# zhen6618/EPRecon

Measured on AMD Instinct MI355X. Metric: fragments_per_sec, higher is better.
Workload: dtype f32

## Files before the change

### eprecon_amd/csrc/back_project.hip

```cpp
#include <stdlib.h>

#include "common.hpp"

namespace {
using namespace ep;


struct BpParams {
    const int32_t *coords;
    int n;
    const float *origin;
    int batch;
    float voxel_size;
    const float *feats_nhwc;
    const float *krcam;
    int V, C, H, W;
    int Cs;
    int min_view;
    float *out_feats;
    float *out_mean;
    int32_t *out_coords;
    float *count;
    float *out_grid;
    uint8_t *out_mask;
    int32_t *n_valid_dev;
    int32_t *block_offsets;
    int xcd_slabs;
};

struct Proj {
    float gx, gy, pz;
    bool vis;
};

__device__ __forceinline__ Proj project(const float *P, float X, float Y, float Z, float wm1,
                                        float hm1)
{
    const float px = __fmaf_rn(P[3], 1.0f, __fmaf_rn(P[2], Z, __fmaf_rn(P[1], Y, __fmul_rn(P[0], X))));
    const float py = __fmaf_rn(P[7], 1.0f, __fmaf_rn(P[6], Z, __fmaf_rn(P[5], Y, __fmul_rn(P[4], X))));
    const float pz = __fmaf_rn(P[11], 1.0f, __fmaf_rn(P[10], Z, __fmaf_rn(P[9], Y, __fmul_rn(P[8], X))));
    const float u = __fdiv_rn(px, pz);
    const float v = __fdiv_rn(py, pz);
    Proj r;
    r.gx = __fsub_rn(__fdiv_rn(__fmul_rn(2.0f, u), wm1), 1.0f);
    r.gy = __fsub_rn(__fdiv_rn(__fmul_rn(2.0f, v), hm1), 1.0f);
    r.pz = pz;
    r.vis = (fabsf(r.gx) <= 1.0f) && (fabsf(r.gy) <= 1.0f) && (pz > 0.0f);
    return r;
}

struct ProjFast {
    float u, v, pz;
    bool vis;
};

__device__ __forceinline__ ProjFast project_fast(const float *P, float X, float Y, float Z, float wm1, float hm1,
                                                 float kx, float ky)
{
    const float px = __fmaf_rn(P[3], 1.0f, __fmaf_rn(P[2], Z, __fmaf_rn(P[1], Y, __fmul_rn(P[0], X))));
    const float py = __fmaf_rn(P[7], 1.0f, __fmaf_rn(P[6], Z, __fmaf_rn(P[5], Y, __fmul_rn(P[4], X))));
    const float pz = __fmaf_rn(P[11], 1.0f, __fmaf_rn(P[10], Z, __fmaf_rn(P[9], Y, __fmul_rn(P[8], X))));
    float r = __builtin_amdgcn_rcpf(pz);
    r = r * fmaf(-pz, r, 2.0f);
    const float u = px * r, v = py * r;
    const float gx = fmaf(u, kx, -1.0f), gy = fmaf(v, ky, -1.0f);
    ProjFast o;
    o.pz = pz;
    const bool near_edge = fabsf(fabsf(gx) - 1.0f) < 1e-4f || fabsf(fabsf(gy) - 1.0f) < 1e-4f;
    if (near_edge) {
        const float ue = __fdiv_rn(px, pz), ve = __fdiv_rn(py, pz);
        const float gxe = __fsub_rn(__fdiv_rn(__fmul_rn(2.0f, ue), wm1), 1.0f);
        const float gye = __fsub_rn(__fdiv_rn(__fmul_rn(2.0f, ve), hm1), 1.0f);
        o.vis = (fabsf(gxe) <= 1.0f) && (fabsf(gye) <= 1.0f) && (pz > 0.0f);
    } else {
        o.vis = (fabsf(gx) <= 1.0f) && (fabsf(gy) <= 1.0f) && (pz > 0.0f);
    }
    o.u = fminf(fmaxf(u, 0.0f), wm1);
    o.v = fminf(fmaxf(v, 0.0f), hm1);
    return o;
}

__device__ __forceinline__ void voxel_centre(const int4 c, const float *origin, float vs, float &X,
                                             float &Y, float &Z)
{
    X = __fadd_rn(__fmul_rn((float)c.y, vs), origin[3 * c.x + 0]);
    Y = __fadd_rn(__fmul_rn((float)c.z, vs), origin[3 * c.x + 1]);
    Z = __fadd_rn(__fmul_rn((float)c.w, vs), origin[3 * c.x + 2]);
}

__device__ __forceinline__ void stage_matrices(float *sP, const float *krcam, int nmat, int tid,
                                               int nthreads)
{
    for (int i = tid; i < nmat * 12; i += nthreads) {
        const int m = i / 12, e = i - m * 12;
        sP[i] = krcam[m * 16 + e];
    }
}

template <int VOX>
__global__ __launch_bounds__(256) void bp_count_kernel(BpParams p, int32_t *tile_sums, int32_t *blk_batch)
{
    constexpr int BLOCK = 256;
    extern __shared__ __attribute__((aligned(16))) char smem[];
    float *sP = reinterpret_cast<float *>(smem);
    int *sBatch = reinterpret_cast<int *>(sP + p.V * p.batch * 12);
    int *sWave = sBatch + p.batch;
    const int tid = threadIdx.x;
    stage_matrices(sP, p.krcam, p.V * p.batch, tid, BLOCK);
    for (int b = tid; b < p.batch; b += BLOCK) sBatch[b] = 0;
    __syncthreads();

    const int i = blockIdx.x * BLOCK + tid;
    bool valid = false;
    int vbatch = 0;
    if (i < p.n) {
        const int4 c = reinterpret_cast<const int4 *>(p.coords)[i];
        int cnt = 0;
        const bool in_range = c.x >= 0 && c.x < p.batch;
        if (in_range) {
            float X, Y, Z;
            voxel_centre(c, p.origin, p.voxel_size, X, Y, Z);
            const float wm1 = (float)(p.W - 1), hm1 = (float)(p.H - 1);
            const float kx = 2.0f / wm1, ky = 2.0f / hm1;
            for (int v = 0; v < p.V; ++v)
                cnt += project_fast(sP + (v * p.batch + c.x) * 12, X, Y, Z, wm1, hm1, kx, ky).vis ? 1 : 0;
        }
        p.count[i] = (float)cnt;
        valid = in_range && cnt >= p.min_view;
        vbatch = c.x;
    }
    const unsigned long long m = __ballot(valid);
    const int lane = tid & (kWave - 1);
    {
        const int b0 = __shfl(vbatch, m ? (__ffsll((long long)m) - 1) : 0);
        const bool uniform = __ballot(valid && vbatch != b0) == 0ull;
        if (uniform) {
            if (m && lane == (__ffsll((long long)m) - 1)) atomicAdd(&sBatch[b0], __popcll(m));
        } else if (valid) {
            atomicAdd(&sBatch[vbatch], 1);
        }
    }
    if constexpr (VOX >= kWave) {
        if (lane == 0) sWave[tid / kWave] = __popcll(m);
        __syncthreads();
        constexpr int WPT = VOX / kWave;
        if (tid < BLOCK / VOX) {
            int t = 0;
            for (int w = 0; w < WPT; ++w) t += sWave[tid * WPT + w];
            const int tile = blockIdx.x * (BLOCK / VOX) + tid;
            if ((long long)tile * VOX < p.n) tile_sums[tile] = t;
        }
    } else {
        if ((lane % VOX) == 0 && i < p.n) tile_sums[i / VOX] = __popcll((m >> lane) & ((1ull << VOX) - 1ull));
        __syncthreads();
    }
    if (blk_batch) {
        __syncthreads();
        for (int b = tid; b < p.batch; b += BLOCK) blk_batch[(size_t)blockIdx.x * p.batch + b] = sBatch[b];
    }
}

__global__ __launch_bounds__(1024) void bp_scan_kernel(int32_t *block_sums, int nblk,
                                                       int32_t *n_valid_dev, const int32_t *blk_batch = nullptr,
                                                       int nblk_count = 0, int batch = 0)
{
    __shared__ int sWave[1024 / kWave];
    const int tid = threadIdx.x, lane = tid & (kWave - 1), wid = tid / kWave;
    int carry = 0;
    for (int base = 0; base < nblk; base += 1024) {
        const int i = base + tid;
        const int v = i < nblk ? block_sums[i] : 0;
        int x = v;
#pragma unroll
        for (int d = 1; d < kWave; d <<= 1) {
            const int y = __shfl_up(x, d);
            if (lane >= d) x += y;
        }
        if (lane == kWave - 1) sWave[wid] = x;
        __syncthreads();
        int woff = 0, tot = 0;
#pragma unroll
        for (int w = 0; w < 1024 / kWave; ++w) {
            const int c = sWave[w];
            woff += (w < wid) ? c : 0;
            tot += c;
        }
        if (i < nblk) block_sums[i] = carry + woff + x - v;
        carry += tot;
        __syncthreads();
    }
    if (tid == 0) n_valid_dev[0] = carry;
    if (batch == 1) {
        if (tid == 0) n_valid_dev[1] = carry;
    } else if (blk_batch) {
        for (int b = 0; b < batch; ++b) {
            int x = 0;
            for (int i = tid; i < nblk_count; i += 1024) x += blk_batch[(size_t)i * batch + b];
#pragma unroll
            for (int d = kWave / 2; d > 0; d >>= 1) x += __shfl_xor(x, d);
            __syncthreads();
            if (lane == 0) sWave[wid] = x;
            __syncthreads();
            if (tid == 0) {
                int t = 0;
                for (int w = 0; w < 1024 / kWave; ++w) t += sWave[w];
                n_valid_dev[1 + b] = t;
            }
        }
    }
}

struct Taps {
    int o00, o10, o01, o11;
    float w00, w10, w01, w11;
};

__device__ __forceinline__ Taps make_taps(float ix, float iy, int W, int H, int C)
{
    const float x0f = floorf(ix), y0f = floorf(iy);
    int x0 = (int)x0f, y0 = (int)y0f;
    float wx1 = ix - x0f, wx0 = (x0f + 1.0f) - ix;
    float wy1 = iy - y0f, wy0 = (y0f + 1.0f) - iy;
    int x1 = x0 + 1, y1 = y0 + 1;
    if (x1 >= W) { x1 = W - 1; wx1 = 0.0f; }
    if (y1 >= H) { y1 = H - 1; wy1 = 0.0f; }
    Taps t;
    t.o00 = (y0 * W + x0) * C;
    t.o10 = (y0 * W + x1) * C;
    t.o01 = (y1 * W + x0) * C;
    t.o11 = (y1 * W + x1) * C;
    t.w00 = wx0 * wy0;
    t.w10 = wx1 * wy0;
    t.w01 = wx0 * wy1;
    t.w11 = wx1 * wy1;
    return t;
}

template <int VEC>
struct Chan;
template <>
struct Chan<4> {
    float4 v;
    __device__ __forceinline__ static Chan zero() { return Chan{make_float4(0.f, 0.f, 0.f, 0.f)}; }
    __device__ __forceinline__ static Chan sample(const float *m, const Taps &t)
    {
        const float4 a = *reinterpret_cast<const float4 *>(m + t.o00);
        const float4 b = *reinterpret_cast<const float4 *>(m + t.o10);
        const float4 c = *reinterpret_cast<const float4 *>(m + t.o01);
        const float4 d = *reinterpret_cast<const float4 *>(m + t.o11);
        Chan r;
        r.v.x = fmaf(d.x, t.w11, fmaf(c.x, t.w01, fmaf(b.x, t.w10, a.x * t.w00)));
        r.v.y = fmaf(d.y, t.w11, fmaf(c.y, t.w01, fmaf(b.y, t.w10, a.y * t.w00)));
        r.v.z = fmaf(d.z, t.w11, fmaf(c.z, t.w01, fmaf(b.z, t.w10, a.z * t.w00)));
        r.v.w = fmaf(d.w, t.w11, fmaf(c.w, t.w01, fmaf(b.w, t.w10, a.w * t.w00)));
        return r;
    }
    __device__ __forceinline__ void add(const Chan &o) { v.x += o.v.x; v.y += o.v.y; v.z += o.v.z; v.w += o.v.w; }
    __device__ __forceinline__ void add_sqdiff(const Chan &f, const Chan &mean)
    {
        const float dx = f.v.x - mean.v.x, dy = f.v.y - mean.v.y, dz = f.v.z - mean.v.z, dw = f.v.w - mean.v.w;
        v.x = fmaf(dx, dx, v.x); v.y = fmaf(dy, dy, v.y); v.z = fmaf(dz, dz, v.z); v.w = fmaf(dw, dw, v.w);
    }
    __device__ __forceinline__ Chan div(float d) const
    {
        return Chan{make_float4(__fdiv_rn(v.x, d), __fdiv_rn(v.y, d), __fdiv_rn(v.z, d), __fdiv_rn(v.w, d))};
    }
    __device__ __forceinline__ void store(float *dst, bool aligned16) const
    {
        if (aligned16) {
            *reinterpret_cast<float4 *>(dst) = v;
        } else {
            dst[0] = v.x; dst[1] = v.y; dst[2] = v.z; dst[3] = v.w;
        }
    }
};
template <>
struct Chan<1> {
    float v;
    __device__ __forceinline__ static Chan zero() { return Chan{0.f}; }
    __device__ __forceinline__ static Chan sample(const float *m, const Taps &t)
    {
        return Chan{fmaf(m[t.o11], t.w11, fmaf(m[t.o01], t.w01, fmaf(m[t.o10], t.w10, m[t.o00] * t.w00)))};
    }
    __device__ __forceinline__ void add(const Chan &o) { v += o.v; }
    __device__ __forceinline__ void add_sqdiff(const Chan &f, const Chan &mean)
    {
        const float d = f.v - mean.v;
        v = fmaf(d, d, v);
    }
    __device__ __forceinline__ Chan div(float d) const { return Chan{__fdiv_rn(v, d)}; }
    __device__ __forceinline__ void store(float *dst, bool) const { dst[0] = v; }
};

template <int VOX, int MODE, int VEC, int QT>
__global__ __launch_bounds__(256) void bp_gather_kernel(BpParams p)
{
    extern __shared__ __attribute__((aligned(16))) char smem[];
    constexpr int BLOCK = 256;
    float2 *sPix = reinterpret_cast<float2 *>(smem);
    float *sP = reinterpret_cast<float *>(sPix + VOX * p.V);
    const int nP = (p.V * p.batch * 12 + 3) & ~3;
    uint32_t *sVis = reinterpret_cast<uint32_t *>(sP + nP);
    float *sDen = reinterpret_cast<float *>(sVis + VOX);
    int *sBatch = reinterpret_cast<int *>(sDen + VOX);
    int *sSlot = sBatch + VOX;
    int *sOut = sSlot + VOX;
    int *sWave = sOut + VOX;

    const int tid = threadIdx.x;
    const int lb = p.xcd_slabs ? xcd_remap(blockIdx.x, gridDim.x) : (int)blockIdx.x;
    stage_matrices(sP, p.krcam, p.V * p.batch, tid, BLOCK);
    __syncthreads();

    const int e = lb * VOX + tid;
    const int i = e;
    const float wm1 = (float)(p.W - 1), hm1 = (float)(p.H - 1);
    bool valid = false;
    int4 c = make_int4(0, 0, 0, 0);
    float X = 0.f, Y = 0.f, Z = 0.f, zsum = 0.f;
    int cnt = 0;
    uint32_t vis = 0;
    if (tid < VOX && e < p.n) {
        c = reinterpret_cast<const int4 *>(p.coords)[i];
        if (c.x >= 0 && c.x < p.batch) {
            voxel_centre(c, p.origin, p.voxel_size, X, Y, Z);
            for (int v = 0; v < p.V; ++v) {
                const Proj pr = project(sP + (v * p.batch + c.x) * 12, X, Y, Z, wm1, hm1);
                const float ix = __fmul_rn(__fdiv_rn(__fadd_rn(pr.gx, 1.0f), 2.0f), wm1);
                const float iy = __fmul_rn(__fdiv_rn(__fadd_rn(pr.gy, 1.0f), 2.0f), hm1);
                sPix[tid * p.V + v] = make_float2(ix, iy);
                if (pr.vis) {
                    vis |= 1u << v;
                    cnt += 1;
                    zsum += pr.pz;
                }
            }
            valid = cnt >= p.min_view;
        }
    }
    int nloc;
    const int rank = block_exclusive_rank<BLOCK>(valid, sWave, nloc);
    if (nloc == 0) return;
    const int base = p.block_offsets[lb];
    const int n_valid = p.n_valid_dev[0];
    const int cout = (MODE == EPRECON_BP_MEAN_DEPTH) ? p.C + 1 : p.C;
    if (valid) {
        const int o = base + rank;
        sSlot[rank] = tid;
        sOut[tid] = o;
        sVis[tid] = vis;
        const float den = (float)(cnt > 0 ? cnt : 1);
        sDen[tid] = den;
        sBatch[tid] = c.x;
        reinterpret_cast<int4 *>(p.out_coords)[o] = c;
        if (MODE == EPRECON_BP_MEAN_DEPTH) p.out_feats[(size_t)o * cout + p.C] = __fdiv_rn(zsum, den);
        if (p.out_grid || p.out_mask) {
            for (int v = 0; v < p.V; ++v) {
                const Proj pr = project(sP + (v * p.batch + c.x) * 12, X, Y, Z, wm1, hm1);
                if (p.out_grid)
                    reinterpret_cast<float2 *>(p.out_grid)[(size_t)v * n_valid + o] = make_float2(pr.gx, pr.gy);
                if (p.out_mask) p.out_mask[(size_t)v * n_valid + o] = pr.vis ? 1 : 0;
            }
        }
    }
    __syncthreads();

    const int Q = QT > 0 ? QT : p.C / VEC;
    const size_t map_elems = (size_t)p.H * p.W * p.Cs;
    const bool aligned16 = (MODE != EPRECON_BP_MEAN_DEPTH);
    for (int w = tid; w < nloc * Q; w += BLOCK) {
        const int r = w / Q;
        const int q = w - r * Q;
        const int t = sSlot[r];
        const uint32_t vm = sVis[t];
        const float den = sDen[t];
        const int b = sBatch[t];
        const float *fb = p.feats_nhwc + (size_t)b * map_elems + q * VEC;
        const size_t vstride = (size_t)p.batch * map_elems;
        Chan<VEC> acc = Chan<VEC>::zero();
        for (int v = 0; v < p.V; ++v) {
            if (vm & (1u << v)) {
                const float2 px = sPix[t * p.V + v];
                const Taps tp = make_taps(px.x, px.y, p.W, p.H, p.Cs);
                acc.add(Chan<VEC>::sample(fb + (size_t)v * vstride, tp));
            }
        }
        const int orow = sOut[t];
        float *dst = p.out_feats + (size_t)orow * cout + q * VEC;
        if (MODE == EPRECON_BP_VARIANCE) {
            const Chan<VEC> mean = acc.div(den);
            Chan<VEC> sq = Chan<VEC>::zero();
            for (int v = 0; v < p.V; ++v) {
                if (vm & (1u << v)) {
                    const float2 px = sPix[t * p.V + v];
                    const Taps tp = make_taps(px.x, px.y, p.W, p.H, p.Cs);
                    sq.add_sqdiff(Chan<VEC>::sample(fb + (size_t)v * vstride, tp), mean);
                }
            }
            sq.div(den).store(dst, true);
            if (p.out_mean) mean.store(p.out_mean + (size_t)orow * p.C + q * VEC, true);
        } else {
            acc.div(den).store(dst, aligned16);
        }
    }
}


typedef unsigned int u32x4 __attribute__((ext_vector_type(4)));

constexpr int kOobOffset = (int)0x80000000u;

template <int U, class F>
__device__ __forceinline__ void visit_visible_samples(__amdgpu_buffer_rsrc_t rsrc, const int *sOffRow,
                                                      const float2 *sWxyRow, uint32_t vm, int qbyte, int s10,
                                                      int s01, int s11, F &&f)
{
    uint32_t m = vm;
    while (m) {
        int off[U];
        float2 wxy[U];
        bool on[U];
#pragma unroll
        for (int u = 0; u < U; ++u) {
            on[u] = m != 0;
            const int v = on[u] ? __builtin_ctz(m) : 0;
            m &= m - 1;
            wxy[u] = sWxyRow[v];
            off[u] = on[u] ? sOffRow[v] + qbyte : kOobOffset;
        }
        u32x4 a[U], b[U], c[U], d[U];
#pragma unroll
        for (int u = 0; u < U; ++u) {
            a[u] = __builtin_amdgcn_raw_buffer_load_b128(rsrc, off[u], 0, 0);
            b[u] = __builtin_amdgcn_raw_buffer_load_b128(rsrc, off[u], s10, 0);
            c[u] = __builtin_amdgcn_raw_buffer_load_b128(rsrc, off[u], s01, 0);
            d[u] = __builtin_amdgcn_raw_buffer_load_b128(rsrc, off[u], s11, 0);
        }
#pragma unroll
        for (int u = 0; u < U; ++u) {
            const float wx1 = wxy[u].x, wy1 = wxy[u].y;
            const float wx0 = 1.0f - wx1, wy0 = 1.0f - wy1;
            const float w00 = wx0 * wy0, w10 = wx1 * wy0, w01 = wx0 * wy1, w11 = wx1 * wy1;
            float4 r;
#define EP_TAP(k) fmaf(__uint_as_float(d[u].k), w11, fmaf(__uint_as_float(c[u].k), w01, fmaf(__uint_as_float(b[u].k), w10, __uint_as_float(a[u].k) * w00)))
            r.x = EP_TAP(x); r.y = EP_TAP(y); r.z = EP_TAP(z); r.w = EP_TAP(w);
#undef EP_TAP
            if (on[u]) f(r);
        }
    }
}

template <int VOX, int MODE, int QT, int U>
__global__ __launch_bounds__(256) void bp_gather_mlp_kernel(BpParams p)
{
    extern __shared__ __attribute__((aligned(16))) char smem[];
    constexpr int BLOCK = 256;
    constexpr int VPT = BLOCK / VOX;
    float2 *sWxy = reinterpret_cast<float2 *>(smem);
    int *sOff = reinterpret_cast<int *>(sWxy + VOX * p.V);
    float *sP = reinterpret_cast<float *>(sOff + VOX * p.V);
    const int nP = (p.V * p.batch * 12 + 3) & ~3;
    uint32_t *sVis = reinterpret_cast<uint32_t *>(sP + nP);
    int *sSlot = reinterpret_cast<int *>(sVis + VOX);
    int *sOut = sSlot + VOX;
    int *sWave = sOut + VOX;

    const int tid = threadIdx.x;
    const int lb = p.xcd_slabs ? xcd_remap(blockIdx.x, gridDim.x) : (int)blockIdx.x;
    stage_matrices(sP, p.krcam, p.V * p.batch, tid, BLOCK);
    if (VPT > 1 && tid < VOX) sVis[tid] = 0;
    __syncthreads();

    const float wm1 = (float)(p.W - 1), hm1 = (float)(p.H - 1);
    const float kx = 2.0f / wm1, ky = 2.0f / hm1;
    const int map_elems = p.H * p.W * p.Cs;
    const int vx = tid % VOX;
    const int e = lb * VOX + vx;
    int4 c = make_int4(-1, 0, 0, 0);
    if (e < p.n) c = reinterpret_cast<const int4 *>(p.coords)[e];
    const bool in_batch = c.x >= 0 && c.x < p.batch;
    uint32_t vis = 0;
    if (in_batch) {
        float X, Y, Z;
        voxel_centre(c, p.origin, p.voxel_size, X, Y, Z);
        for (int v = tid / VOX; v < p.V; v += VPT) {
            const ProjFast q = project_fast(sP + (v * p.batch + c.x) * 12, X, Y, Z, wm1, hm1, kx, ky);
            if (!q.vis) continue;
            const float x0f = fminf(floorf(q.u), wm1 - 1.0f), y0f = fminf(floorf(q.v), hm1 - 1.0f);
            sWxy[vx * p.V + v] = make_float2(q.u - x0f, q.v - y0f);
            sOff[vx * p.V + v] = ((v * p.batch + c.x) * map_elems + ((int)y0f * p.W + (int)x0f) * p.Cs) * 4;
            vis |= 1u << v;
        }
        if (VPT > 1 && vis) atomicOr(&sVis[vx], vis);
    }
    if (VPT > 1) {
        __syncthreads();
        vis = sVis[vx];
    }
    const int cnt = __popc(vis);
    const bool valid = tid < VOX && in_batch && cnt >= p.min_view;
    int nloc;
    const int rank = block_exclusive_rank<BLOCK>(valid, sWave, nloc);
    if (nloc == 0) return;
    const int n_valid = p.n_valid_dev[0];
    const int cout = (MODE == EPRECON_BP_MEAN_DEPTH) ? p.C + 1 : p.C;
    if (valid) {
        const int o = p.block_offsets[lb] + rank;
        sSlot[rank] = tid;
        sOut[tid] = o;
        if (VPT == 1) sVis[tid] = vis;
        reinterpret_cast<int4 *>(p.out_coords)[o] = c;
        if (MODE == EPRECON_BP_MEAN_DEPTH || p.out_grid || p.out_mask) {
            float X, Y, Z, zsum = 0.0f;
            voxel_centre(c, p.origin, p.voxel_size, X, Y, Z);
            for (int v = 0; v < p.V; ++v) {
                const Proj pr = project(sP + (v * p.batch + c.x) * 12, X, Y, Z, wm1, hm1);
                if (pr.vis) zsum += pr.pz;
                if (p.out_grid)
                    reinterpret_cast<float2 *>(p.out_grid)[(size_t)v * n_valid + o] = make_float2(pr.gx, pr.gy);
                if (p.out_mask) p.out_mask[(size_t)v * n_valid + o] = pr.vis ? 1 : 0;
            }
            if (MODE == EPRECON_BP_MEAN_DEPTH)
                p.out_feats[(size_t)o * cout + p.C] = __fdiv_rn(zsum, (float)(cnt > 0 ? cnt : 1));
        }
    }
    __syncthreads();
    const __amdgpu_buffer_rsrc_t rsrc = __builtin_amdgcn_make_buffer_rsrc(
        const_cast<float *>(p.feats_nhwc), 0, p.V * p.batch * map_elems * 4, 0x00020000);
    const int Q = QT > 0 ? QT : p.C / 4;
    const int s10 = p.Cs * 4, s01 = p.W * p.Cs * 4, s11 = s01 + s10;
    for (int w = tid; w < nloc * Q; w += BLOCK) {
        const int r = w / Q, q = w - r * Q;
        const int t = sSlot[r];
        const uint32_t vm = sVis[t];
        const float den = (float)max(__popc(vm), 1);
        const int *offRow = sOff + t * p.V;
        const float2 *wxyRow = sWxy + t * p.V;
        float4 acc = make_float4(0.f, 0.f, 0.f, 0.f);
        visit_visible_samples<U>(rsrc, offRow, wxyRow, vm, q * 16, s10, s01, s11, [&](const float4 &f) {
            acc.x += f.x; acc.y += f.y; acc.z += f.z; acc.w += f.w;
        });
        const int orow = sOut[t];
        float *dst = p.out_feats + (size_t)orow * cout + q * 4;
        const float4 mean = make_float4(__fdiv_rn(acc.x, den), __fdiv_rn(acc.y, den), __fdiv_rn(acc.z, den),
                                        __fdiv_rn(acc.w, den));
        if (MODE == EPRECON_BP_VARIANCE) {
            float4 sq = make_float4(0.f, 0.f, 0.f, 0.f);
            visit_visible_samples<U>(rsrc, offRow, wxyRow, vm, q * 16, s10, s01, s11, [&](const float4 &f) {
                const float dx = f.x - mean.x, dy = f.y - mean.y, dz = f.z - mean.z, dw = f.w - mean.w;
                sq.x = fmaf(dx, dx, sq.x); sq.y = fmaf(dy, dy, sq.y); sq.z = fmaf(dz, dz, sq.z); sq.w = fmaf(dw, dw, sq.w);
            });
            *reinterpret_cast<float4 *>(dst) = make_float4(__fdiv_rn(sq.x, den), __fdiv_rn(sq.y, den),
                                                           __fdiv_rn(sq.z, den), __fdiv_rn(sq.w, den));
            if (p.out_mean) *reinterpret_cast<float4 *>(p.out_mean + (size_t)orow * p.C + q * 4) = mean;
        } else if (MODE == EPRECON_BP_MEAN_DEPTH) {
            dst[0] = mean.x; dst[1] = mean.y; dst[2] = mean.z; dst[3] = mean.w;
        } else {
            *reinterpret_cast<float4 *>(dst) = mean;
        }
    }
}


__global__ __launch_bounds__(1024) void bp_depth_norm_kernel(float *out_feats, int cout,
                                                             const int32_t *n_valid_dev)
{
    __shared__ float sRed[1024 / kWave];
    __shared__ float sBcast[2];
    const int b = blockIdx.x, tid = threadIdx.x, lane = tid & (kWave - 1), wid = tid / kWave;
    int start = 0;
    for (int k = 0; k < b; ++k) start += n_valid_dev[1 + k];
    const int len = n_valid_dev[1 + b];
    float *d = out_feats + (size_t)start * cout + (cout - 1);

    auto block_sum = [&](float x) -> float {
#pragma unroll
        for (int s = kWave / 2; s > 0; s >>= 1) x += __shfl_xor(x, s);
        __syncthreads();
        if (lane == 0) sRed[wid] = x;
        __syncthreads();
        float t = 0.f;
#pragma unroll
        for (int w = 0; w < 1024 / kWave; ++w) t += sRed[w];
        return t;
    };
    float s = 0.f, m = 0.f;
    for (int j = tid; j < len; j += 1024) {
        const float x = d[(size_t)j * cout];
        if (x > 0.f) { s += x; m += 1.f; }
    }
    const float tot = block_sum(s), cntp = block_sum(m);
    const float mu = tot / cntp;
    float ss = 0.f;
    for (int j = tid; j < len; j += 1024) {
        const float x = d[(size_t)j * cout];
        if (x > 0.f) ss = fmaf(x - mu, x - mu, ss);
    }
    const float sigma = sqrtf(block_sum(ss)) + 1e-5f;
    for (int j = tid; j < len; j += 1024) {
        const float x = d[(size_t)j * cout];
        d[(size_t)j * cout] = x > 0.f ? (x - mu) / sigma : 0.f;
    }
    (void)sBcast;
}

constexpr int kTrPix = 64;
__global__ __launch_bounds__(256) void nchw_to_nhwc_kernel(const float *__restrict__ in,
                                                           float *__restrict__ out, int C, int hw, int Cs,
                                                           int32_t *zero = nullptr, int zero_n = 0)
{
    extern __shared__ __attribute__((aligned(16))) char smem[];
    float *tile = reinterpret_cast<float *>(smem);
    if (blockIdx.x == 0 && blockIdx.y == 0 && (int)threadIdx.x < zero_n) zero[threadIdx.x] = 0;
    const int map = blockIdx.y;
    const int p0 = blockIdx.x * kTrPix;
    const int npix = min(kTrPix, hw - p0);
    const float *src = in + (size_t)map * C * hw;
    float *dst = out + (size_t)map * hw * Cs + (size_t)p0 * Cs;
    for (int e = threadIdx.x; e < C * kTrPix; e += 256) {
        const int c = e / kTrPix, px = e - c * kTrPix;
        if (px < npix) tile[c * (kTrPix + 1) + px] = src[(size_t)c * hw + p0 + px];
    }
    __syncthreads();
    for (int e = threadIdx.x; e < npix * Cs; e += 256) {
        const int px = e / Cs, c = e - px * Cs;
        dst[e] = c < C ? tile[c * (kTrPix + 1) + px] : 0.0f;
    }
}


struct ViewsParams {
    eprecon_views_desc d;
    int tile0[4];
    int tiles[3];
};
__global__ __launch_bounds__(256) void views_to_rows_kernel(ViewsParams p)
{
    extern __shared__ __attribute__((aligned(16))) char smem[];
    float *tile = reinterpret_cast<float *>(smem);
    const int b = blockIdx.x;
    const int l = b >= p.tile0[2] ? 2 : (b >= p.tile0[1] ? 1 : 0);
    const int r = b - p.tile0[l];
    const int v = r / p.tiles[l], t = r - v * p.tiles[l];
    const int C = p.d.channels[l], hw = p.d.hw[l];
    const int p0 = t * kTrPix;
    const int npix = min(kTrPix, hw - p0);
    const float *src = p.d.src[l][v];
    float *dst = p.d.dst[l] + ((size_t)v * hw + p0) * C;
    for (int e = threadIdx.x; e < C * kTrPix; e += 256) {
        const int c = e / kTrPix, px = e - c * kTrPix;
        if (px < npix) tile[c * (kTrPix + 1) + px] = src[(size_t)c * hw + p0 + px];
    }
    __syncthreads();
    for (int e = threadIdx.x; e < npix * C; e += 256) {
        const int px = e / C, c = e - px * C;
        dst[e] = tile[c * (kTrPix + 1) + px];
    }
}

struct BpBwdParams {
    const int32_t *coords; int64_t n;
    const float *origin; int batch; float voxel_size;
    const float *feats_nhwc; const float *krcam;
    int V, C, H, W, mode;
    const float *dout; int ld_dout;
    const float *dmean;
    float *dfeats;
    unsigned long long *dfix;
};

constexpr double kFixScale = 1099511627776.0;
__device__ __forceinline__ unsigned long long to_fixed(float v)
{
    const double x = fmin(fmax((double)v * kFixScale, -9.0e18), 9.0e18);
    return (unsigned long long)__double2ll_rn(x);
}
constexpr float kFixMax = 8.0e6f;
__device__ __forceinline__ void fixed_add(unsigned long long *acc, float *mark, float v)
{
// ... 30 lines not shown
    float mean = 0.0f;
    if (p.mode == EPRECON_BP_VARIANCE) {
        for (int v = 0; v < p.V; ++v) {
            const Proj pr = project(sP + (v * p.batch + c.x) * 12, X, Y, Z, wm1, hm1);
            if (!pr.vis) continue;
            const float ix = __fmul_rn(__fdiv_rn(__fadd_rn(pr.gx, 1.0f), 2.0f), wm1);
            const float iy = __fmul_rn(__fdiv_rn(__fadd_rn(pr.gy, 1.0f), 2.0f), hm1);
            mean += Chan<1>::sample(p.feats_nhwc + ((size_t)v * p.batch + c.x) * map_elems + ch, make_taps(ix, iy, p.W, p.H, p.C)).v;
        }
        mean *= inv;
    }
    const float gm = (p.mode == EPRECON_BP_VARIANCE && p.dmean) ? p.dmean[i * p.C + ch] * inv : 0.0f;
    for (int v = 0; v < p.V; ++v) {
        const Proj pr = project(sP + (v * p.batch + c.x) * 12, X, Y, Z, wm1, hm1);
        if (!pr.vis) continue;
        const float ix = __fmul_rn(__fdiv_rn(__fadd_rn(pr.gx, 1.0f), 2.0f), wm1);
        const float iy = __fmul_rn(__fdiv_rn(__fadd_rn(pr.gy, 1.0f), 2.0f), hm1);
        const Taps t = make_taps(ix, iy, p.W, p.H, p.C);
        const size_t mo = ((size_t)v * p.batch + c.x) * map_elems + ch;
        float gv;
        if (p.mode == EPRECON_BP_VARIANCE) {
            const float f = Chan<1>::sample(p.feats_nhwc + mo, t).v;
            gv = 2.0f * (f - mean) * inv * g + gm;
        } else {
            gv = g * inv;
        }
        if (p.dfix) {
            unsigned long long *d = p.dfix + mo;
            float *m = p.dfeats + mo;
            if (t.w00 != 0.0f) fixed_add(d + t.o00, m + t.o00, t.w00 * gv);
            if (t.w10 != 0.0f) fixed_add(d + t.o10, m + t.o10, t.w10 * gv);
            if (t.w01 != 0.0f) fixed_add(d + t.o01, m + t.o01, t.w01 * gv);
            if (t.w11 != 0.0f) fixed_add(d + t.o11, m + t.o11, t.w11 * gv);
        } else {
            float *d = p.dfeats + mo;
            if (t.w00 != 0.0f) unsafeAtomicAdd(d + t.o00, t.w00 * gv);
            if (t.w10 != 0.0f) unsafeAtomicAdd(d + t.o10, t.w10 * gv);
            if (t.w01 != 0.0f) unsafeAtomicAdd(d + t.o01, t.w01 * gv);
            if (t.w11 != 0.0f) unsafeAtomicAdd(d + t.o11, t.w11 * gv);
        }
    }
}

struct ProfileState {
    bool on = false, recorded = false, one_shot = false;
    hipEvent_t start = nullptr, stop = nullptr;
    const char *kernel = "";
} g_prof;

size_t gather_lds_bytes(int vox, int V, int B)
{
    const size_t nP = ((size_t)V * B * 12 + 3) & ~(size_t)3;
    return (size_t)vox * V * sizeof(float2) + nP * sizeof(float) + (size_t)vox * 5 * 4 +
           (size_t)(256 / kWave) * 4 + 16;
}

template <int VOX, int MODE>
int launch_gather(const BpParams &p, int nblk, hipStream_t st)
{
    const size_t lds = gather_lds_bytes(VOX, p.V, p.batch);
    const dim3 grid(nblk), block(256);
#define EP_GATHER(VEC, QT) hipLaunchKernelGGL((bp_gather_kernel<VOX, MODE, VEC, QT>), grid, block, lds, st, p)
    if (p.C % 4 == 0) {
        switch (p.C / 4) {
            case 6: EP_GATHER(4, 6); break;
            case 8: EP_GATHER(4, 8); break;
            case 10: EP_GATHER(4, 10); break;
            case 20: EP_GATHER(4, 20); break;
            default: EP_GATHER(4, 0); break;
        }
    } else {
        EP_GATHER(1, 0);
    }
#undef EP_GATHER
    EP_LAUNCH_CHECK();
    return EPRECON_OK;
}

size_t gather_mlp_lds_bytes(int vox, int V, int B)
{
    const size_t nP = ((size_t)V * B * 12 + 3) & ~(size_t)3;
    return (size_t)vox * V * 12 + nP * sizeof(float) + (size_t)vox * 3 * 4 + (size_t)(256 / kWave) * 4 + 16;
}

size_t gather_lds_limit()
{
    static const size_t limit = [] {
        int dev = 0, v = 0;
        if (hipGetDevice(&dev) != hipSuccess ||
            hipDeviceGetAttribute(&v, hipDeviceAttributeMaxSharedMemoryPerBlock, dev) != hipSuccess || v <= 0)
            v = 64 * 1024;
        return (size_t)(v < 64 * 1024 ? v : 64 * 1024);
    }();
    return limit;
}

bool gather_mlp_supported(const BpParams &p)
{
    return p.C % 4 == 0 && p.Cs % 4 == 0 && p.V <= 32 &&
           (size_t)p.V * p.batch * p.H * p.W * p.Cs * 4 < 0x7fff0000ull &&
           gather_mlp_lds_bytes(256, p.V, p.batch) <= gather_lds_limit();
}

template <int VOX, int MODE, int U>
int launch_gather_mlp_u(const BpParams &p, int nblk, hipStream_t st)
{
    const size_t lds = gather_mlp_lds_bytes(VOX, p.V, p.batch);
    const dim3 grid(nblk), block(256);
#define EP_GATHER(QT) hipLaunchKernelGGL((bp_gather_mlp_kernel<VOX, MODE, QT, U>), grid, block, lds, st, p)
    switch (p.C / 4) {
        case 6: EP_GATHER(6); break;
        case 8: EP_GATHER(8); break;
        case 10: EP_GATHER(10); break;
        case 20: EP_GATHER(20); break;
        default: EP_GATHER(0); break;
    }
#undef EP_GATHER
    EP_LAUNCH_CHECK();
    return EPRECON_OK;
}

template <int VOX, int MODE>
int launch_gather_mlp(const BpParams &p, int nblk, hipStream_t st)
{
    return launch_gather_mlp_u<VOX, MODE, 1>(p, nblk, st);
}

}

namespace ep {
int profile_bracket_begin(hipStream_t st)
{
    if (g_prof.on && g_prof.start) EP_HIP_CHECK(hipEventRecord(g_prof.start, st));
    return EPRECON_OK;
}
// ... 4 lines not shown
        g_prof.recorded = true;
        g_prof.kernel = kernel;
        if (g_prof.one_shot) g_prof.on = false;
    }
    return EPRECON_OK;
}
}

extern "C" {

const char *eprecon_profile_gather_kernel(void) { return g_prof.kernel; }

int eprecon_abi_version(void) { return EPRECON_ABI_VERSION; }
const char *eprecon_build_arch(void) { return "gfx950"; }

size_t eprecon_back_project_workspace_bytes(int64_t n, int batch, int n_views, int channels,
                                            int height, int width, int feats_layout)
{
    size_t bytes = ep::align_up((size_t)ep::ceil_div(n > 0 ? n : 1, 16) * sizeof(int32_t), 256);
    bytes += ep::align_up((size_t)ep::ceil_div(n > 0 ? n : 1, 256) * (batch > 0 ? batch : 1) * sizeof(int32_t), 256);
    if (feats_layout == EPRECON_LAYOUT_NCHW)
        bytes += ep::align_up((size_t)n_views * batch * channels * height * width * sizeof(float), 256);
    return bytes + 256;
}

int eprecon_profile_enable(int on)
{
    if (on && !g_prof.start) {
        EP_HIP_CHECK(hipEventCreate(&g_prof.start));
        EP_HIP_CHECK(hipEventCreate(&g_prof.stop));
    }
    g_prof.on = on != 0;
    g_prof.one_shot = on == 2;
    if (on != 0) g_prof.recorded = false;
    return EPRECON_OK;
}

float eprecon_profile_gather_ms(void)
{
    if (!g_prof.recorded) return -1.0f;
    if (hipEventSynchronize(g_prof.stop) != hipSuccess) return -1.0f;
    float ms = -1.0f;
    if (hipEventElapsedTime(&ms, g_prof.start, g_prof.stop) != hipSuccess) return -1.0f;
    return ms;
}

int eprecon_nchw_to_nhwc_async(const float *in, float *out, int maps, int channels, int hw,
                               void *stream)
{
    if (!in || !out || maps <= 0 || channels <= 0 || hw <= 0) return EPRECON_ERR_ARG;
    const size_t lds = (size_t)channels * (kTrPix + 1) * sizeof(float);
    if (lds > 64 * 1024) return EPRECON_ERR_UNSUPPORTED;
    const dim3 grid((unsigned)ep::ceil_div(hw, kTrPix), (unsigned)maps);
    hipLaunchKernelGGL(nchw_to_nhwc_kernel, grid, dim3(256), lds, (hipStream_t)stream, in, out,
                       channels, hw, channels);
    EP_LAUNCH_CHECK();
    return EPRECON_OK;
}

int eprecon_views_to_rows_async(const eprecon_views_desc *desc, void *stream)
{
    if (!desc || desc->levels < 1 || desc->levels > 3 || desc->n_views < 1 || desc->n_views > 16) return EPRECON_ERR_ARG;
    ViewsParams p = {};
    p.d = *desc;
    int cmax = 0, at = 0;
    for (int l = 0; l < 3; ++l) {
        p.tile0[l] = at;
        if (l >= desc->levels) { p.tiles[l] = 1; continue; }
        if (desc->channels[l] <= 0 || desc->hw[l] <= 0 || !desc->dst[l]) return EPRECON_ERR_ARG;
        for (int v = 0; v < desc->n_views; ++v)
            if (!desc->src[l][v]) return EPRECON_ERR_ARG;
        p.tiles[l] = ep::ceil_div(desc->hw[l], kTrPix);
        at += p.tiles[l] * desc->n_views;
        cmax = desc->channels[l] > cmax ? desc->channels[l] : cmax;
    }
    p.tile0[3] = at;
    for (int l = desc->levels; l < 3; ++l) p.tile0[l] = at;
    const size_t lds = (size_t)cmax * (kTrPix + 1) * sizeof(float);
    if (lds > 64 * 1024) return EPRECON_ERR_UNSUPPORTED;
    hipLaunchKernelGGL(views_to_rows_kernel, dim3((unsigned)at), dim3(256), lds, (hipStream_t)stream, p);
    EP_LAUNCH_CHECK();
    return EPRECON_OK;
}

int eprecon_back_project_async(const int32_t *coords, int64_t n, const float *origin, int batch,
                               float voxel_size, const float *feats, int feats_layout,
                               const float *krcam, int n_views, int channels, int height,
                               int width, int min_view, int mode, float *out_feats,
                               float *out_mean, int32_t *out_coords, float *count,
                               float *out_grid, uint8_t *out_mask, int32_t *n_valid_dev,
                               void *workspace, size_t workspace_bytes, void *stream)
{
    hipStream_t st = (hipStream_t)stream;
    if (n < 0 || n > 0x7fffffff / 64 || batch <= 0 || n_views <= 0 || n_views > 32 || channels <= 0 ||
        height <= 1 || width <= 1 || mode < 0 || mode > 2)
        return EPRECON_ERR_ARG;
    if (!origin || !feats || !krcam || !n_valid_dev || !workspace) return EPRECON_ERR_ARG;
    if (n > 0 && (!coords || !out_feats || !out_coords || !count)) return EPRECON_ERR_ARG;
    if ((size_t)n_views * batch * 12 * sizeof(float) > 32 * 1024) return EPRECON_ERR_UNSUPPORTED;
    if (workspace_bytes < eprecon_back_project_workspace_bytes(n, batch, n_views, channels, height,
                                                               width, feats_layout))
        return EPRECON_ERR_WORKSPACE;
    if ((size_t)n_views * batch * channels * height * width > 0x7fffffffull) return EPRECON_ERR_UNSUPPORTED;

    const bool clear_in_relayout = n > 0 && feats_layout == EPRECON_LAYOUT_NCHW && batch < 256;
    if (!clear_in_relayout) EP_HIP_CHECK(hipMemsetAsync(n_valid_dev, 0, sizeof(int32_t) * (size_t)(1 + batch), st));
    if (n == 0) return EPRECON_OK;

    char *ws = reinterpret_cast<char *>(workspace);
    int32_t *block_sums = reinterpret_cast<int32_t *>(ws);
    ws += ep::align_up((size_t)ep::ceil_div(n, 16) * sizeof(int32_t), 256);
    int32_t *blk_batch = reinterpret_cast<int32_t *>(ws);
    ws += ep::align_up((size_t)ep::ceil_div(n, 256) * batch * sizeof(int32_t), 256);
    const float *nhwc = feats;
    int pix_stride = channels;
    if (feats_layout == EPRECON_LAYOUT_NCHW) {
        float *tmp = reinterpret_cast<float *>(ws);
        const size_t lds_t = (size_t)channels * (kTrPix + 1) * sizeof(float);
        if (lds_t > 64 * 1024) return EPRECON_ERR_UNSUPPORTED;
        hipLaunchKernelGGL(nchw_to_nhwc_kernel, dim3((unsigned)ep::ceil_div(height * width, kTrPix), (unsigned)(n_views * batch)),
                           dim3(256), lds_t, st, feats, tmp, channels, height * width, pix_stride, n_valid_dev, 1 + batch);
        EP_LAUNCH_CHECK();
        nhwc = tmp;
        ws += ep::align_up((size_t)n_views * batch * pix_stride * height * width * sizeof(float), 256);
    } else if (feats_layout != EPRECON_LAYOUT_NHWC) {
        return EPRECON_ERR_ARG;
    }

    BpParams p;
    p.coords = coords; p.n = (int)n; p.origin = origin; p.batch = batch; p.voxel_size = voxel_size;
    p.feats_nhwc = nhwc; p.krcam = krcam; p.V = n_views; p.C = channels; p.Cs = pix_stride; p.H = height; p.W = width;
    p.min_view = min_view; p.out_feats = out_feats; p.out_mean = out_mean; p.out_coords = out_coords;
    p.count = count; p.out_grid = out_grid; p.out_mask = out_mask; p.n_valid_dev = n_valid_dev;
    p.block_offsets = block_sums;
    {
        const char *e = getenv("EPRECON_BP_XCD_SLABS");
        p.xcd_slabs = (e && e[0] == '0') ? 0 : 1;
    }

    int vox = n >= 512 * 1024 ? 256 : (n >= 48 * 1024 ? 64 : 16);
    if (vox == 256 && !gather_mlp_supported(p) && gather_lds_bytes(256, n_views, batch) > gather_lds_limit()) vox = 64;
    const int ntile = (int)ep::ceil_div(n, vox);
    const int nblk_count = (int)ep::ceil_div(n, 256);
    const size_t lds_count = ((size_t)n_views * batch * 12 + batch + 256 / ep::kWave) * 4 + 16;
    int32_t *bb = batch > 1 ? blk_batch : nullptr;
    if (vox == 256)
        hipLaunchKernelGGL((bp_count_kernel<256>), dim3(nblk_count), dim3(256), lds_count, st, p, block_sums, bb);
    else if (vox == 64)
        hipLaunchKernelGGL((bp_count_kernel<64>), dim3(nblk_count), dim3(256), lds_count, st, p, block_sums, bb);
    else
        hipLaunchKernelGGL((bp_count_kernel<16>), dim3(nblk_count), dim3(256), lds_count, st, p, block_sums, bb);
    EP_LAUNCH_CHECK();
    hipLaunchKernelGGL(bp_scan_kernel, dim3(1), dim3(1024), 0, st, block_sums, ntile, n_valid_dev,
                       (const int32_t *)bb, nblk_count, batch);
    EP_LAUNCH_CHECK();

    const bool prof = g_prof.on && g_prof.start;
    if (prof) EP_HIP_CHECK(hipEventRecord(g_prof.start, st));
    int rc;
#define EP_MODE_DISPATCH(VOX)                                                                        \
    rc = mode == EPRECON_BP_MEAN ? launch_gather<VOX, EPRECON_BP_MEAN>(p, ntile, st)                   \
       : mode == EPRECON_BP_MEAN_DEPTH ? launch_gather<VOX, EPRECON_BP_MEAN_DEPTH>(p, ntile, st)       \
                                       : launch_gather<VOX, EPRECON_BP_VARIANCE>(p, ntile, st)
#define EP_MODE_DISPATCH_MLP(VOX)                                                                    \
    rc = mode == EPRECON_BP_MEAN ? launch_gather_mlp<VOX, EPRECON_BP_MEAN>(p, ntile, st)               \
       : mode == EPRECON_BP_MEAN_DEPTH ? launch_gather_mlp<VOX, EPRECON_BP_MEAN_DEPTH>(p, ntile, st)   \
                                       : launch_gather_mlp<VOX, EPRECON_BP_VARIANCE>(p, ntile, st)
    if (gather_mlp_supported(p)) {
        if (vox == 256) { EP_MODE_DISPATCH_MLP(256); }
        else if (vox == 64) { EP_MODE_DISPATCH_MLP(64); }
        else { EP_MODE_DISPATCH_MLP(16); }
    }
    else if (vox == 256) { EP_MODE_DISPATCH(256); }
    else if (vox == 64) { EP_MODE_DISPATCH(64); }
    else { EP_MODE_DISPATCH(16); }
#undef EP_MODE_DISPATCH
#undef EP_MODE_DISPATCH_MLP
    if (rc != EPRECON_OK) return rc;
    if (prof) {
        EP_HIP_CHECK(hipEventRecord(g_prof.stop, st));
        g_prof.recorded = true;
        g_prof.kernel = gather_mlp_supported(p) ? "bp_gather_mlp_kernel" : "bp_gather_kernel";
        if (g_prof.one_shot) g_prof.on = false;
    }
    if (mode == EPRECON_BP_MEAN_DEPTH) {
        hipLaunchKernelGGL(bp_depth_norm_kernel, dim3(batch), dim3(1024), 0, st, out_feats,
                           channels + 1, n_valid_dev);
        EP_LAUNCH_CHECK();
    }
    return EPRECON_OK;
}

int eprecon_back_project(const int32_t *coords, int64_t n, const float *origin, int batch,
                         float voxel_size, const float *feats, int feats_layout,
                         const float *krcam, int n_views, int channels, int height, int width,
                         int min_view, int mode, int min_valid_per_batch, float *out_feats,
                         float *out_mean, int32_t *out_coords, float *count, float *out_grid,
                         uint8_t *out_mask, int32_t *n_valid_dev, int32_t *n_valid_host,
                         void *workspace, size_t workspace_bytes, void *stream)
{
    if (!n_valid_host) return EPRECON_ERR_ARG;
    const int rc = eprecon_back_project_async(coords, n, origin, batch, voxel_size, feats, feats_layout,
                                              krcam, n_views, channels, height, width, min_view, mode,
                                              out_feats, out_mean, out_coords, count, out_grid, out_mask,
                                              n_valid_dev, workspace, workspace_bytes, stream);
    if (rc != EPRECON_OK) return rc;
    hipStream_t st = (hipStream_t)stream;
    EP_HIP_CHECK(hipMemcpyAsync(n_valid_host, n_valid_dev, sizeof(int32_t) * (size_t)(1 + batch),
// ... 63 lines not shown
```

Baseline: 737.6.

## Fuse relayout with count kernel and fold tile scan into gather blocks

Merges the NCHW-to-NHWC relayout and the per-voxel visibility count into one prepare kernel. When the tile count is below a cap, the separate single-block scan kernel is removed: each gather block sums the preceding tile counts itself, and the last block writes the totals. Also adds a float4-vectorized relayout path. The aim is fewer kernel launches and serialized small kernels, at the cost of redundant prefix-sum reads in every gather block and more LDS per block.

```diff
diff --git a/eprecon_amd/csrc/back_project.hip b/eprecon_amd/csrc/back_project.hip
--- a/eprecon_amd/csrc/back_project.hip
+++ b/eprecon_amd/csrc/back_project.hip
@@ -25,6 +25,10 @@
     uint8_t *out_mask;
     int32_t *n_valid_dev;
     int32_t *block_offsets;
+    int fold;
+    int ntile;
+    const int32_t *blk_batch;
+    int nblk_count;
     int xcd_slabs;
 };
 
@@ -98,10 +102,9 @@
 }
 
 template <int VOX>
-__global__ __launch_bounds__(256) void bp_count_kernel(BpParams p, int32_t *tile_sums, int32_t *blk_batch)
+__device__ __forceinline__ void count_body(char *smem, const BpParams &p, int32_t *tile_sums, int32_t *blk_batch, int bid)
 {
     constexpr int BLOCK = 256;
-    extern __shared__ __attribute__((aligned(16))) char smem[];
     float *sP = reinterpret_cast<float *>(smem);
     int *sBatch = reinterpret_cast<int *>(sP + p.V * p.batch * 12);
     int *sWave = sBatch + p.batch;
@@ -110,7 +113,7 @@
     for (int b = tid; b < p.batch; b += BLOCK) sBatch[b] = 0;
     __syncthreads();
 
-    const int i = blockIdx.x * BLOCK + tid;
+    const int i = bid * BLOCK + tid;
     bool valid = false;
     int vbatch = 0;
     if (i < p.n) {
@@ -147,7 +150,7 @@
         if (tid < BLOCK / VOX) {
             int t = 0;
             for (int w = 0; w < WPT; ++w) t += sWave[tid * WPT + w];
-            const int tile = blockIdx.x * (BLOCK / VOX) + tid;
+            const int tile = bid * (BLOCK / VOX) + tid;
             if ((long long)tile * VOX < p.n) tile_sums[tile] = t;
         }
     } else {
@@ -156,8 +159,15 @@
     }
     if (blk_batch) {
         __syncthreads();
-        for (int b = tid; b < p.batch; b += BLOCK) blk_batch[(size_t)blockIdx.x * p.batch + b] = sBatch[b];
-    }
+        for (int b = tid; b < p.batch; b += BLOCK) blk_batch[(size_t)bid * p.batch + b] = sBatch[b];
+    }
+}
+
+template <int VOX>
+__global__ __launch_bounds__(256) void bp_count_kernel(BpParams p, int32_t *tile_sums, int32_t *blk_batch)
+{
+    extern __shared__ __attribute__((aligned(16))) char smem[];
+    count_body<VOX>(smem, p, tile_sums, blk_batch, (int)blockIdx.x);
 }
 
 __global__ __launch_bounds__(1024) void bp_scan_kernel(int32_t *block_sums, int nblk,
@@ -208,6 +218,73 @@
             }
         }
     }
+}
+
+struct TileBase {
+    int base, n_valid;
+};
+
+__device__ __forceinline__ bool tile_base_all(const BpParams &p, int lb)
+{
+    return p.out_grid != nullptr || p.out_mask != nullptr || lb == p.ntile - 1;
+}
+
+__device__ __forceinline__ void tile_base_partials(const BpParams &p, int lb, int *sFold)
+{
+    constexpr int BLOCK = 256;
+    const int tid = threadIdx.x, lane = tid & (kWave - 1), wid = tid / kWave;
+    const int end = tile_base_all(p, lb) ? p.ntile : lb;
+    int acc = 0, tot = 0;
+#pragma unroll 4
+    for (int t = tid; t < end; t += BLOCK) {
+        const int x = p.block_offsets[t];
+        tot += x;
+        acc += t < lb ? x : 0;
+    }
+#pragma unroll
+    for (int d = kWave / 2; d > 0; d >>= 1) {
+        acc += __shfl_xor(acc, d);
+        tot += __shfl_xor(tot, d);
+    }
+    if (lane == 0) {
+        sFold[wid] = acc;
+        sFold[BLOCK / kWave + wid] = tot;
+    }
+}
+
+__device__ __forceinline__ TileBase tile_base_finish(const BpParams &p, int lb, int *sFold)
+{
+    constexpr int BLOCK = 256, NW = BLOCK / kWave;
+    const int tid = threadIdx.x, lane = tid & (kWave - 1), wid = tid / kWave;
+    TileBase r = {0, 0};
+#pragma unroll
+    for (int w = 0; w < NW; ++w) {
+        r.base += sFold[w];
+        r.n_valid += sFold[NW + w];
+    }
+    if (lb == p.ntile - 1) {
+        if (tid == 0) {
+            p.n_valid_dev[0] = r.n_valid;
+            if (p.batch == 1) p.n_valid_dev[1] = r.n_valid;
+        }
+        if (p.batch > 1 && p.blk_batch) {
+            for (int b = 0; b < p.batch; ++b) {
+                int x = 0;
+                for (int i = tid; i < p.nblk_count; i += BLOCK) x += p.blk_batch[(size_t)i * p.batch + b];
+#pragma unroll
+                for (int d = kWave / 2; d > 0; d >>= 1) x += __shfl_xor(x, d);
+                __syncthreads();
+                if (lane == 0) sFold[wid] = x;
+                __syncthreads();
+                if (tid == 0) {
+                    int t = 0;
+                    for (int w = 0; w < NW; ++w) t += sFold[w];
+                    p.n_valid_dev[1 + b] = t;
+                }
+            }
+        }
+    }
+    return r;
 }
 
 struct Taps {
@@ -306,10 +383,12 @@
     int *sSlot = sBatch + VOX;
     int *sOut = sSlot + VOX;
     int *sWave = sOut + VOX;
+    int *sFold = sWave + BLOCK / kWave;
 
     const int tid = threadIdx.x;
     const int lb = p.xcd_slabs ? xcd_remap(blockIdx.x, gridDim.x) : (int)blockIdx.x;
     stage_matrices(sP, p.krcam, p.V * p.batch, tid, BLOCK);
+    if (p.fold) tile_base_partials(p, lb, sFold);
     __syncthreads();
 
     const int e = lb * VOX + tid;
@@ -340,9 +419,11 @@
     }
     int nloc;
     const int rank = block_exclusive_rank<BLOCK>(valid, sWave, nloc);
+    TileBase tb = {0, 0};
+    if (p.fold) tb = tile_base_finish(p, lb, sFold);
     if (nloc == 0) return;
-    const int base = p.block_offsets[lb];
-    const int n_valid = p.n_valid_dev[0];
+    const int base = p.fold ? tb.base : p.block_offsets[lb];
+    const int n_valid = p.fold ? tb.n_valid : p.n_valid_dev[0];
     const int cout = (MODE == EPRECON_BP_MEAN_DEPTH) ? p.C + 1 : p.C;
     if (valid) {
         const int o = base + rank;
@@ -408,6 +489,8 @@
 
 typedef unsigned int u32x4 __attribute__((ext_vector_type(4)));
 
+constexpr int kFoldCapDefault = 6144;
+
 constexpr int kOobOffset = (int)0x80000000u;
 
 template <int U, class F>
@@ -464,11 +547,13 @@
     int *sSlot = reinterpret_cast<int *>(sVis + VOX);
     int *sOut = sSlot + VOX;
     int *sWave = sOut + VOX;
+    int *sFold = sWave + BLOCK / kWave;
 
     const int tid = threadIdx.x;
     const int lb = p.xcd_slabs ? xcd_remap(blockIdx.x, gridDim.x) : (int)blockIdx.x;
     stage_matrices(sP, p.krcam, p.V * p.batch, tid, BLOCK);
     if (VPT > 1 && tid < VOX) sVis[tid] = 0;
+    if (p.fold) tile_base_partials(p, lb, sFold);
     __syncthreads();
 
     const float wm1 = (float)(p.W - 1), hm1 = (float)(p.H - 1);
@@ -501,11 +586,13 @@
     const bool valid = tid < VOX && in_batch && cnt >= p.min_view;
     int nloc;
     const int rank = block_exclusive_rank<BLOCK>(valid, sWave, nloc);
+    TileBase tb = {0, 0};
+    if (p.fold) tb = tile_base_finish(p, lb, sFold);
     if (nloc == 0) return;
-    const int n_valid = p.n_valid_dev[0];
+    const int n_valid = p.fold ? tb.n_valid : p.n_valid_dev[0];
     const int cout = (MODE == EPRECON_BP_MEAN_DEPTH) ? p.C + 1 : p.C;
     if (valid) {
-        const int o = p.block_offsets[lb] + rank;
+        const int o = (p.fold ? tb.base : p.block_offsets[lb]) + rank;
         sSlot[rank] = tid;
         sOut[tid] = o;
         if (VPT == 1) sVis[tid] = vis;
@@ -605,26 +692,76 @@
 }
 
 constexpr int kTrPix = 64;
+template <bool VEC4>
+__device__ __forceinline__ void relayout_body(char *smem, const float *__restrict__ in, float *__restrict__ out, int C, int hw,
+                                              int Cs, int map, int p0)
+{
+    float *tile = reinterpret_cast<float *>(smem);
+    const int npix = min(kTrPix, hw - p0);
+    const float *src = in + (size_t)map * C * hw;
+    float *dst = out + (size_t)map * hw * Cs + (size_t)p0 * Cs;
+    if constexpr (VEC4) {
+        constexpr int G = kTrPix / 4;
+        for (int e = threadIdx.x; e < C * G; e += 256) {
+            const int c = e / G, px = (e - c * G) * 4;
+            if (px < npix) {
+                const float4 v = *reinterpret_cast<const float4 *>(src + (size_t)c * hw + p0 + px);
+                float *t = tile + c * (kTrPix + 1) + px;
+                t[0] = v.x; t[1] = v.y; t[2] = v.z; t[3] = v.w;
+            }
+        }
+        __syncthreads();
+        const int Q = Cs / 4;
+        for (int e = threadIdx.x; e < npix * Q; e += 256) {
+            const int px = e / Q, c = (e - px * Q) * 4;
+            const float *t = tile + c * (kTrPix + 1) + px;
+            float4 v;
+            v.x = c + 0 < C ? t[0 * (kTrPix + 1)] : 0.0f;
+            v.y = c + 1 < C ? t[1 * (kTrPix + 1)] : 0.0f;
+            v.z = c + 2 < C ? t[2 * (kTrPix + 1)] : 0.0f;
+            v.w = c + 3 < C ? t[3 * (kTrPix + 1)] : 0.0f;
+            reinterpret_cast<float4 *>(dst)[e] = v;
+        }
+    } else {
+        for (int e = threadIdx.x; e < C * kTrPix; e += 256) {
+            const int c = e / kTrPix, px = e - c * kTrPix;
+            if (px < npix) tile[c * (kTrPix + 1) + px] = src[(size_t)c * hw + p0 + px];
+        }
+        __syncthreads();
+        for (int e = threadIdx.x; e < npix * Cs; e += 256) {
+            const int px = e / Cs, c = e - px * Cs;
+            dst[e] = c < C ? tile[c * (kTrPix + 1) + px] : 0.0f;
+        }
+    }
+}
+
+bool relayout_vec4(const void *in, const void *out, int hw, int Cs)
+{
+    return hw % 4 == 0 && Cs % 4 == 0 && (((uintptr_t)in | (uintptr_t)out) & 15) == 0;
+}
+
+template <bool VEC4>
 __global__ __launch_bounds__(256) void nchw_to_nhwc_kernel(const float *__restrict__ in,
                                                            float *__restrict__ out, int C, int hw, int Cs,
                                                            int32_t *zero = nullptr, int zero_n = 0)
 {
     extern __shared__ __attribute__((aligned(16))) char smem[];
-    float *tile = reinterpret_cast<float *>(smem);
     if (blockIdx.x == 0 && blockIdx.y == 0 && (int)threadIdx.x < zero_n) zero[threadIdx.x] = 0;
-    const int map = blockIdx.y;
-    const int p0 = blockIdx.x * kTrPix;
-    const int npix = min(kTrPix, hw - p0);
-    const float *src = in + (size_t)map * C * hw;
-    float *dst = out + (size_t)map * hw * Cs + (size_t)p0 * Cs;
-    for (int e = threadIdx.x; e < C * kTrPix; e += 256) {
-        const int c = e / kTrPix, px = e - c * kTrPix;
-        if (px < npix) tile[c * (kTrPix + 1) + px] = src[(size_t)c * hw + p0 + px];
-    }
-    __syncthreads();
-    for (int e = threadIdx.x; e < npix * Cs; e += 256) {
-        const int px = e / Cs, c = e - px * Cs;
-        dst[e] = c < C ? tile[c * (kTrPix + 1) + px] : 0.0f;
+    relayout_body<VEC4>(smem, in, out, C, hw, Cs, (int)blockIdx.y, (int)blockIdx.x * kTrPix);
+}
+
+template <int VOX, bool VEC4>
+__global__ __launch_bounds__(256) void bp_prepare_kernel(BpParams p, int32_t *tile_sums, int32_t *blk_batch,
+                                                         const float *__restrict__ in, float *__restrict__ out, int hw,
+                                                         int tiles, int R)
+{
+    extern __shared__ __attribute__((aligned(16))) char smem[];
+    const int bid = blockIdx.x;
+    if (bid < R) {
+        const int map = bid / tiles;
+        relayout_body<VEC4>(smem, in, out, p.C, hw, p.Cs, map, (bid - map * tiles) * kTrPix);
+    } else {
+        count_body<VOX>(smem, p, tile_sums, blk_batch, bid - R);
     }
 }
 
@@ -761,7 +898,7 @@
 {
     const size_t nP = ((size_t)V * B * 12 + 3) & ~(size_t)3;
     return (size_t)vox * V * sizeof(float2) + nP * sizeof(float) + (size_t)vox * 5 * 4 +
-           (size_t)(256 / kWave) * 4 + 16;
+           (size_t)(256 / kWave) * 4 * 3;
 }
 
 template <int VOX, int MODE>
@@ -789,7 +926,7 @@
 size_t gather_mlp_lds_bytes(int vox, int V, int B)
 {
     const size_t nP = ((size_t)V * B * 12 + 3) & ~(size_t)3;
-    return (size_t)vox * V * 12 + nP * sizeof(float) + (size_t)vox * 3 * 4 + (size_t)(256 / kWave) * 4 + 16;
+    return (size_t)vox * V * 12 + nP * sizeof(float) + (size_t)vox * 3 * 4 + (size_t)(256 / kWave) * 4 * 3;
 }
 
 size_t gather_lds_limit()
@@ -900,8 +1037,12 @@
     const size_t lds = (size_t)channels * (kTrPix + 1) * sizeof(float);
     if (lds > 64 * 1024) return EPRECON_ERR_UNSUPPORTED;
     const dim3 grid((unsigned)ep::ceil_div(hw, kTrPix), (unsigned)maps);
-    hipLaunchKernelGGL(nchw_to_nhwc_kernel, grid, dim3(256), lds, (hipStream_t)stream, in, out,
-                       channels, hw, channels);
+    if (relayout_vec4(in, out, hw, channels))
+        hipLaunchKernelGGL(nchw_to_nhwc_kernel<true>, grid, dim3(256), lds, (hipStream_t)stream, in, out, channels, hw, channels,
+                           (int32_t *)nullptr, 0);
+    else
+        hipLaunchKernelGGL(nchw_to_nhwc_kernel<false>, grid, dim3(256), lds, (hipStream_t)stream, in, out, channels, hw, channels,
+                           (int32_t *)nullptr, 0);
     EP_LAUNCH_CHECK();
     return EPRECON_OK;
 }
@@ -951,8 +1092,17 @@
         return EPRECON_ERR_WORKSPACE;
     if ((size_t)n_views * batch * channels * height * width > 0x7fffffffull) return EPRECON_ERR_UNSUPPORTED;
 
-    const bool clear_in_relayout = n > 0 && feats_layout == EPRECON_LAYOUT_NCHW && batch < 256;
-    if (!clear_in_relayout) EP_HIP_CHECK(hipMemsetAsync(n_valid_dev, 0, sizeof(int32_t) * (size_t)(1 + batch), st));
+    if (feats_layout != EPRECON_LAYOUT_NCHW && feats_layout != EPRECON_LAYOUT_NHWC) return EPRECON_ERR_ARG;
+    const bool nchw = feats_layout == EPRECON_LAYOUT_NCHW;
+    int fold_cap = kFoldCapDefault;
+    if (const char *e = getenv("EPRECON_BP_FOLD"); e && e[0]) {
+        const long v = strtol(e, nullptr, 10);
+        fold_cap = v <= 0 ? 0 : (v > 0x7fffffffL ? 0x7fffffff : (int)v);
+    }
+    const bool chain4 = fold_cap == 0;
+    const bool clear_in_relayout = chain4 && n > 0 && nchw && batch < 256;
+    if (n == 0 || (chain4 && !clear_in_relayout))
+        EP_HIP_CHECK(hipMemsetAsync(n_valid_dev, 0, sizeof(int32_t) * (size_t)(1 + batch), st));
     if (n == 0) return EPRECON_OK;
 
     char *ws = reinterpret_cast<char *>(workspace);
@@ -960,24 +1110,14 @@
     ws += ep::align_up((size_t)ep::ceil_div(n, 16) * sizeof(int32_t), 256);
     int32_t *blk_batch = reinterpret_cast<int32_t *>(ws);
     ws += ep::align_up((size_t)ep::ceil_div(n, 256) * batch * sizeof(int32_t), 256);
-    const float *nhwc = feats;
-    int pix_stride = channels;
-    if (feats_layout == EPRECON_LAYOUT_NCHW) {
-        float *tmp = reinterpret_cast<float *>(ws);
-        const size_t lds_t = (size_t)channels * (kTrPix + 1) * sizeof(float);
-        if (lds_t > 64 * 1024) return EPRECON_ERR_UNSUPPORTED;
-        hipLaunchKernelGGL(nchw_to_nhwc_kernel, dim3((unsigned)ep::ceil_div(height * width, kTrPix), (unsigned)(n_views * batch)),
-                           dim3(256), lds_t, st, feats, tmp, channels, height * width, pix_stride, n_valid_dev, 1 + batch);
-        EP_LAUNCH_CHECK();
-        nhwc = tmp;
-        ws += ep::align_up((size_t)n_views * batch * pix_stride * height * width * sizeof(float), 256);
-    } else if (feats_layout != EPRECON_LAYOUT_NHWC) {
-        return EPRECON_ERR_ARG;
-    }
+    const int pix_stride = channels;
+    float *tmp = reinterpret_cast<float *>(ws);
+    const size_t lds_t = (size_t)channels * (kTrPix + 1) * sizeof(float);
+    if (nchw && lds_t > 64 * 1024) return EPRECON_ERR_UNSUPPORTED;
 
     BpParams p;
     p.coords = coords; p.n = (int)n; p.origin = origin; p.batch = batch; p.voxel_size = voxel_size;
-    p.feats_nhwc = nhwc; p.krcam = krcam; p.V = n_views; p.C = channels; p.Cs = pix_stride; p.H = height; p.W = width;
+    p.feats_nhwc = nchw ? tmp : feats; p.krcam = krcam; p.V = n_views; p.C = channels; p.Cs = pix_stride; p.H = height; p.W = width;
     p.min_view = min_view; p.out_feats = out_feats; p.out_mean = out_mean; p.out_coords = out_coords;
     p.count = count; p.out_grid = out_grid; p.out_mask = out_mask; p.n_valid_dev = n_valid_dev;
     p.block_offsets = block_sums;
@@ -992,16 +1132,42 @@
     const int nblk_count = (int)ep::ceil_div(n, 256);
     const size_t lds_count = ((size_t)n_views * batch * 12 + batch + 256 / ep::kWave) * 4 + 16;
     int32_t *bb = batch > 1 ? blk_batch : nullptr;
-    if (vox == 256)
-        hipLaunchKernelGGL((bp_count_kernel<256>), dim3(nblk_count), dim3(256), lds_count, st, p, block_sums, bb);
-    else if (vox == 64)
-        hipLaunchKernelGGL((bp_count_kernel<64>), dim3(nblk_count), dim3(256), lds_count, st, p, block_sums, bb);
-    else
-        hipLaunchKernelGGL((bp_count_kernel<16>), dim3(nblk_count), dim3(256), lds_count, st, p, block_sums, bb);
-    EP_LAUNCH_CHECK();
-    hipLaunchKernelGGL(bp_scan_kernel, dim3(1), dim3(1024), 0, st, block_sums, ntile, n_valid_dev,
-                       (const int32_t *)bb, nblk_count, batch);
-    EP_LAUNCH_CHECK();
+    p.fold = (!chain4 && ntile <= fold_cap) ? 1 : 0;
+    p.ntile = ntile; p.blk_batch = bb; p.nblk_count = nblk_count;
+
+    if (nchw && !chain4) {
+        const int hw = height * width, tiles = ep::ceil_div(hw, kTrPix), R = tiles * n_views * batch;
+        const size_t lds_p = lds_t > lds_count ? lds_t : lds_count;
+        const dim3 grid((unsigned)(R + nblk_count));
+        const bool v4 = relayout_vec4(feats, tmp, hw, pix_stride);
+#define EP_PREPARE(VOX)                                                                                                          \
+    if (v4) hipLaunchKernelGGL((bp_prepare_kernel<VOX, true>), grid, dim3(256), lds_p, st, p, block_sums, bb, feats, tmp, hw, tiles, R); \
+    else hipLaunchKernelGGL((bp_prepare_kernel<VOX, false>), grid, dim3(256), lds_p, st, p, block_sums, bb, feats, tmp, hw, tiles, R)
+        if (vox == 256) { EP_PREPARE(256); }
+        else if (vox == 64) { EP_PREPARE(64); }
+        else { EP_PREPARE(16); }
+#undef EP_PREPARE
+        EP_LAUNCH_CHECK();
+    } else {
+        if (nchw) {
+            hipLaunchKernelGGL(nchw_to_nhwc_kernel<false>, dim3((unsigned)ep::ceil_div(height * width, kTrPix), (unsigned)(n_views * batch)),
+                               dim3(256), lds_t, st, feats, tmp, channels, height * width, pix_stride,
+                               clear_in_relayout ? n_valid_dev : (int32_t *)nullptr, clear_in_relayout ? 1 + batch : 0);
+            EP_LAUNCH_CHECK();
+        }
+        if (vox == 256)
+            hipLaunchKernelGGL((bp_count_kernel<256>), dim3(nblk_count), dim3(256), lds_count, st, p, block_sums, bb);
+        else if (vox == 64)
+            hipLaunchKernelGGL((bp_count_kernel<64>), dim3(nblk_count), dim3(256), lds_count, st, p, block_sums, bb);
+        else
+            hipLaunchKernelGGL((bp_count_kernel<16>), dim3(nblk_count), dim3(256), lds_count, st, p, block_sums, bb);
+        EP_LAUNCH_CHECK();
+    }
+    if (!p.fold) {
+        hipLaunchKernelGGL(bp_scan_kernel, dim3(1), dim3(1024), 0, st, block_sums, ntile, n_valid_dev,
+                           (const int32_t *)bb, nblk_count, batch);
+        EP_LAUNCH_CHECK();
+    }
 
     const bool prof = g_prof.on && g_prof.start;
     if (prof) EP_HIP_CHECK(hipEventRecord(g_prof.start, st));
```

Result: faster. 760.2 (median of 6 runs) (+3.1%).
